# yandooo/cilium

Measured on AMD Instinct MI355X. Metric: L7 verdicts/sec + scanned GB/s (HBM roofline frac), 1/2/4/8 MI355X, higher is better.
Workload: dtype u8

## Files before the change

cilium_amd/_lib.py:

```python
import ctypes as C
import os

HERE = os.path.dirname(os.path.abspath(__file__))
LIB_PATH = os.environ.get("L7G_LIB") or os.path.join(HERE, "libl7gpu.so")

DENY, ALLOW, PARSE_ERROR, INCOMPLETE, UNSUPPORTED = 0, 1, 2, 3, 4
PROTO_HTTP, PROTO_KAFKA, PROTO_MEMCACHE, PROTO_R2D2, PROTO_CASSANDRA = 1, 2, 3, 4, 5
VERDICT_NAMES = {DENY: "DENY", ALLOW: "ALLOW", PARSE_ERROR: "PARSE_ERROR",
                 INCOMPLETE: "INCOMPLETE", UNSUPPORTED: "UNSUPPORTED"}


class Conn(C.Structure):
    _fields_ = [("policy", C.c_int32), ("port", C.c_uint32), ("ingress", C.c_uint8),
                ("proto", C.c_uint8), ("flags", C.c_uint16), ("src_id", C.c_uint32),
                ("dst_id", C.c_uint32)]


class Stats(C.Structure):
    _fields_ = [(n, C.c_uint32) for n in (
        "policies", "rules", "http_rulesets", "http_chunks", "http_dfas", "http_dfa_states",
        "kafka_rulesets", "kafka_rules", "kafka_topics")] + [
        ("table_bytes", C.c_uint64), ("http_image_bytes", C.c_uint64), ("hot_ruleset", C.c_int32),
        ("hot_image_bytes", C.c_uint32)] + [
        (n, C.c_uint32) for n in ("mc_rulesets", "mc_rules", "mc_dfas", "mc_dfa_states", "http_nfas", "mc_nfas")] + [
        ("nfa_pool_bytes", C.c_uint64), ("r2d2_rulesets", C.c_uint32), ("r2d2_rules", C.c_uint32)]


EXPORTS = (
    "l7g_engine_create", "l7g_engine_destroy", "l7g_policy_update", "l7g_policy_index",
    "l7g_policy_nrules", "l7g_conns_set", "l7g_conn_update", "l7g_classify", "l7g_classify_host", "l7g_stats",
    "l7g_debug_regex", "l7g_debug_phase_times", "l7g_profile_enable", "l7g_profile_last",
    "l7g_debug_kafka_phase_times", "l7g_debug_frame_phase_times", "l7g_kafka_deny_response", "l7g_debug_regex_nfa", "l7g_policy_update_proto", "l7g_kafka_corr_create", "l7g_kafka_corr_destroy",
    "l7g_kafka_corr_requests", "l7g_kafka_corr_responses", "l7g_kafka_corr_gc", "l7g_kafka_corr_size",
    "l7g_flow_stats_enable", "l7g_flow_stats",
    "l7g_tables_export", "l7g_tables_import", "l7g_tables_compiled", "l7g_tables_digest",
    "l7g_frame_streams", "l7g_classify_streams", "l7g_service_enable", "l7g_service_stats",
    "l7g_cass_sessions_enable", "l7g_cass_replies", "l7g_cass_replies_host", "l7g_cass_session_reset",
    "l7g_cass_session_stats",
    "l7g_classify_logged", "l7g_classify_logged_host", "l7g_kafka_api_key_name",
    "l7g_deny_replies", "l7g_deny_replies_host", "l7g_deny_reply_template",
)


class FlowStat(C.Structure):
    _fields_ = [("policy", C.c_int32), ("proto", C.c_uint8), ("ingress", C.c_uint8), ("port", C.c_uint16),
                ("received", C.c_uint64), ("forwarded", C.c_uint64), ("denied", C.c_uint64), ("error", C.c_uint64)]


class Span(C.Structure):
    _fields_ = [("off", C.c_uint32), ("len", C.c_uint32)]


class _LogHttp(C.Structure):
    _fields_ = [(n, C.c_uint32) for n in ("method_len", "path_len", "host_off", "host_len", "head_len", "nheaders")]


class _LogKafka(C.Structure):
    _fields_ = [("api_version", C.c_int16), ("pad", C.c_int16), ("correlation_id", C.c_int32),
                ("ntopics", C.c_uint32)]


class _LogUnion(C.Union):
    _fields_ = [("http", _LogHttp), ("kafka", _LogKafka)]


class LogRec(C.Structure):
    _fields_ = [("kind", C.c_uint8), ("flags", C.c_uint8), ("api_key", C.c_int16), ("u", _LogUnion),
                ("reserved", C.c_uint32)]


class LogOut(C.Structure):
    _fields_ = [("rec", C.c_void_p), ("topics", C.c_void_p), ("topic_stride", C.c_uint32)]

# ... 53 lines not shown
    lib.l7g_service_stats.argtypes = [vp, C.POINTER(C.c_uint64)]
    lib.l7g_service_stats.restype = None
    lib.l7g_stats.argtypes = [vp, C.POINTER(Stats)]
    lib.l7g_debug_regex.argtypes = [cp, sz, C.c_int, cp, sz, cp, sz]
    lib.l7g_debug_regex_nfa.argtypes = [cp, sz, C.c_int, cp, sz, cp, sz]
    lib.l7g_debug_phase_times.argtypes = [vp, vp, C.c_int]
    lib.l7g_debug_kafka_phase_times.argtypes = [vp, vp, C.c_int]
    lib.l7g_debug_frame_phase_times.argtypes = [vp, vp, C.c_int]
    lib.l7g_kafka_corr_create.restype = vp
    lib.l7g_kafka_corr_destroy.argtypes = [vp]
    lib.l7g_kafka_corr_requests.argtypes = [vp, vp, vp, vp, C.c_uint32, vp]
    lib.l7g_kafka_corr_responses.argtypes = [vp, vp, vp, vp, C.c_uint32, vp]
    lib.l7g_kafka_corr_gc.restype = C.c_uint64
    lib.l7g_kafka_corr_gc.argtypes = [vp, C.c_uint64]
    lib.l7g_kafka_corr_size.restype = C.c_uint64
    lib.l7g_kafka_corr_size.argtypes = [vp]
    lib.l7g_kafka_deny_response.argtypes = [cp, sz, vp, sz, C.POINTER(C.c_size_t)]
    lib.l7g_profile_enable.argtypes = [vp, C.c_int]
    lib.l7g_flow_stats_enable.argtypes = [vp, C.c_int]
    lib.l7g_flow_stats.argtypes = [vp, vp, C.c_uint32, C.POINTER(C.c_uint32), C.c_int]
    lib.l7g_profile_last.argtypes = [vp, vp]
    if hasattr(lib, "l7g_classify_logged"):
        lib.l7g_classify_logged.argtypes = [vp, vp, C.c_uint64, vp, vp, vp, C.c_uint32, vp, vp, vp, vp,
                                            C.POINTER(LogOut), vp]
        lib.l7g_classify_logged_host.argtypes = [vp, vp, C.c_uint64, vp, vp, vp, C.c_uint32, vp, vp, vp,
                                                 C.POINTER(LogOut)]
        lib.l7g_kafka_api_key_name.restype = cp
        lib.l7g_kafka_api_key_name.argtypes = [C.c_int16]
    if hasattr(lib, "l7g_deny_replies"):
        lib.l7g_deny_replies.argtypes = [vp, vp, C.c_uint64, vp, vp, vp, C.c_uint32, vp, C.POINTER(ReplyOut), vp]
        lib.l7g_deny_replies_host.argtypes = [vp, vp, C.c_uint64, vp, vp, vp, C.c_uint32, vp, C.POINTER(ReplyOut)]
        lib.l7g_deny_reply_template.restype = vp
        lib.l7g_deny_reply_template.argtypes = [C.c_int, C.POINTER(C.c_size_t)]
    _libs[path] = lib
    return lib


def debug_regex(pattern, data, anchored=True, nfa=False):
    lib = load()
    p = pattern.encode() if isinstance(pattern, str) else pattern
    d = data.encode() if isinstance(data, str) else data
    err = C.create_string_buffer(512)
    fn = lib.l7g_debug_regex_nfa if nfa else lib.l7g_debug_regex
    r = fn(p, len(p), 1 if anchored else 0, d, len(d), err, 512)
    if r < 0:
        raise ValueError(err.value.decode(errors="replace"))
    return bool(r)


def kafka_api_key_name(key):
    r = load().l7g_kafka_api_key_name(int(key))
    return r.decode() if r is not None else None


def deny_reply_template(proto):
    n = C.c_size_t(0)
    p = load().l7g_deny_reply_template(int(proto), C.byref(n))
    return C.string_at(p, n.value) if p else b""


def kafka_deny_response(req):
    lib = load()
    cap = 4 * len(req) + 256
    out = C.create_string_buffer(cap)
    n = C.c_size_t(0)
    rc = lib.l7g_kafka_deny_response(req, len(req), out, cap, C.byref(n))
    if rc == -1:
        return None
# ... 40 lines not shown
```

cilium_amd/csrc/capi.cc:

```cpp
#include <algorithm>
#include <cstring>

#include "engine/nfa_pool.h"
#include "engine_state.h"
#include "policy/npds_proto.h"
#include "regex/nfa_walk.h"
#include "regex/re_dfa.h"

namespace {

void set_err(char *err, size_t errlen, const std::string &m) {
    if (!err || errlen == 0) return;
    size_t n = std::min(errlen - 1, m.size());
    memcpy(err, m.data(), n);
    err[n] = 0;
}

template <class T>
size_t Put(std::vector<uint8_t> &blob, const std::vector<T> &v) {
    size_t off = (blob.size() + 255) & ~(size_t)255;
    blob.resize(off + v.size() * sizeof(T) + 16);
    if (!v.empty()) memcpy(blob.data() + off, v.data(), v.size() * sizeof(T));
    return off;
}
// ... 132 lines not shown
        std::vector<uint8_t> blob;
        const BlobLayout L = AssembleBlob(e, blob);
        const HttpImage &H = e->hc->image();
        const KafkaImage &K = e->kc->image();
        const McImage &M = e->mc->image();
        const R2Image &R = e->r2->image();
        const CassImage &CI = e->cs->image();
        uint8_t *d = nullptr;
        if ((rc = hipMalloc(&d, blob.size())) != hipSuccess) return rc;
        if ((rc = hipMemcpy(d, blob.data(), blob.size(), hipMemcpyHostToDevice)) != hipSuccess) { hipFree(d); return rc; }
        if (e->d_blob) { WaitLastClassify(e); hipFree(e->d_blob); }
        e->d_blob = d;
        e->blob_bytes = blob.size();
        HttpTables &T = e->ht;
        T.rulesets = (const DevRuleset *)(d + L.o_rs);
        T.images = d + L.o_img;
        T.nrulesets = (uint32_t)H.rulesets.size();
        T.hot_ruleset = e->hot_ruleset;
        T.nfa_pool = H.nfa_pool.empty() ? nullptr : d + L.o_nfa;
        T.nfa_bits = nullptr;
        auto lane_words = [](uint32_t w) { return w > (uint32_t)kNfaMaxWords ? 2 * w : 0u; };
        T.nfa_scratch = nullptr;
        T.nfa_lane_words = lane_words(e->hc->nfa_max_words());
        KafkaTables &KT = e->kt;
        KT.rulesets = (const DevKafkaRuleset *)(d + L.k_rs);
        KT.rules = (const DevKafkaRule *)(d + L.k_r);
        KT.index = (const uint32_t *)(d + L.k_idx);
        KT.topic_hash = (const DevStrSlot *)(d + L.k_th);
        KT.client_hash = (const DevStrSlot *)(d + L.k_ch);
        KT.strings = (const uint8_t *)(d + L.k_s);
        KT.nrulesets = (uint32_t)K.rulesets.size();
        KT.topic_mask = K.topic_mask;
        KT.client_mask = K.client_mask;
        McTables &MT = e->mt;
        MT.rulesets = (const DevRuleset *)(d + L.m_rs);
        MT.images = d + L.m_img;
        MT.nrulesets = (uint32_t)M.rulesets.size();
        MT.images_len = (uint32_t)M.images.size();
        MT.nfa_pool = M.nfa_pool.empty() ? nullptr : d + L.m_nfa;
        MT.max_chunks = (uint32_t)M.max_chunks;
        MT.nfa_scratch = nullptr;
        MT.nfa_lane_words = lane_words(e->mc->nfa_max_words());
        R2Tables &RT = e->rt;
        RT.rulesets = (const DevRuleset *)(d + L.r_rs);
        RT.images = d + L.r_img;
        RT.nrulesets = (uint32_t)R.rulesets.size();
        RT.nfa_pool = R.nfa_pool.empty() ? nullptr : d + L.r_nfa;
        RT.nfa_scratch = nullptr;
        RT.nfa_lane_words = lane_words(e->r2->nfa_max_words());
        CassTables &CT = e->ct;
        CT.rulesets = (const DevRuleset *)(d + L.c_rs);
        CT.images = d + L.c_img;
        CT.nrulesets = (uint32_t)CI.rulesets.size();
        CT.nfa_pool = CI.nfa_pool.empty() ? nullptr : d + L.c_nfa;
        CT.lower = (const uint32_t *)(d + L.c_low);
        CT.nlower = (uint32_t)(CI.lower.size() / 2);
        CT.nfa_scratch = nullptr;
        CT.nfa_lane_words = lane_words(e->cs->nfa_max_words());
        e->tables_dirty = false;
    }
    if (e->conns_dirty) {
        if ((rc = WaitLastClassify(e)) != hipSuccess) return rc;
        size_t need = std::max<size_t>(e->conns.size(), 1);
        if (need > e->conns_cap) {
            if (e->d_conns) { hipFree(e->d_conns); e->d_conns = nullptr; }
            if ((rc = hipMalloc(&e->d_conns, need * sizeof(DevConn))) != hipSuccess) return rc;
// ... 408 lines not shown
    return (int)rc;
}

int l7g_profile_last(l7g_engine *e, float out_ms[4]) {
    std::lock_guard<std::mutex> g(e->mu);
    for (int k = 0; k < 4; k++) out_ms[k] = 0.f;
    bool any = false;
    for (auto &kv : e->scr) any = any || kv.second->launched;
    if (!e->profile || !any) return (int)hipErrorNotReady;
    hipError_t rc = hipEventSynchronize(e->prof_ev[4]);
    for (int k = 0; k < 4 && rc == hipSuccess; k++)
        if (e->prof_ran[k]) rc = hipEventElapsedTime(&out_ms[k], e->prof_ev[k], e->prof_ev[k + 1]);
    return (int)rc;
}

int l7g_debug_phase_times(l7g_engine *e, uint64_t *out16, int reset) {
    if (!e || e->device < 0) return (int)hipErrorNoDevice;
    hipSetDevice(e->device);
    return (int)HttpPhaseTimes(out16, reset != 0);
}

int l7g_debug_frame_phase_times(l7g_engine *e, uint64_t *out8, int reset) {
    if (!e || e->device < 0) return (int)hipErrorNoDevice;
    hipSetDevice(e->device);
    return (int)FramePhaseTimes(out8, reset != 0);
}

int l7g_debug_kafka_phase_times(l7g_engine *e, uint64_t *out8, int reset) {
    if (!e || e->device < 0) return (int)hipErrorNoDevice;
    hipSetDevice(e->device);
    return (int)KafkaPhaseTimes(out8, reset != 0);
}

int l7g_debug_regex(const char *pat, size_t patlen, int anchored, const uint8_t *s, size_t slen, char *err,
                    size_t errlen) {
    std::string m;
    auto ast = re::Parse(std::string(pat, patlen), &m);
    if (!ast) { set_err(err, errlen, m); return -1; }
    re::DFA d;
    std::vector<re::Pattern> ps{{ast.get(), anchored != 0}};
    if (!re::BuildDFA(ps, 1 << 16, &d, &m)) { set_err(err, errlen, m); return -1; }
    auto acc = re::RunDFA(d, s, slen);
    return (int)(acc[0] & 1);
}

int l7g_debug_regex_nfa(const char *pat, size_t patlen, int anchored, const uint8_t *s, size_t slen, char *err,
                        size_t errlen) {
    std::string m;
    auto ast = re::Parse(std::string(pat, patlen), &m);
    if (!ast) { set_err(err, errlen, m); return -1; }
    re::BitNfa n;
    if (!re::BuildBitNfa({ast.get(), anchored != 0}, kNfaMaxPositions, &n, &m, kNfaMaxWords)) {
        set_err(err, errlen, m);
        return -1;
    }
    std::vector<uint8_t> pool;
    const uint64_t off = AppendDevNfa(n, &pool, &m);
    if (off == ~0ull) { set_err(err, errlen, m); return -1; }
    std::vector<uint64_t> scratch(2 * (size_t)n.W);
    return nfa_run(pool.data(), off, s, (uint32_t)slen, scratch.data()) ? 1 : 0;
}

}
```

cilium_amd/csrc/device_tables.h:

```cpp
#pragma once
#include <stddef.h>
#include <stdint.h>

#if defined(__HIPCC__)
#define L7_HD __host__ __device__
#else
#define L7_HD
#endif

namespace l7 {

enum : uint8_t {
    V_DENY = 0, V_ALLOW = 1, V_PARSE_ERROR = 2, V_INCOMPLETE = 3, V_UNSUPPORTED = 4,
};
enum : uint8_t { PROTO_NONE = 0, PROTO_HTTP = 1, PROTO_KAFKA = 2, PROTO_MEMCACHE = 3, PROTO_R2D2 = 4, PROTO_CASSANDRA = 5 };
#define L7_PROTO_OWNED(p) ((p) >= PROTO_HTTP && (p) <= PROTO_CASSANDRA)

#ifndef L7_KAFKA_CLASSES
#define L7_KAFKA_CLASSES 8
#endif

constexpr int kCntWords = 32;
constexpr int kCntMc = L7_KAFKA_CLASSES;
constexpr int kCntHttp = L7_KAFKA_CLASSES + 2;
// ... 133 lines not shown
    uint64_t nfa;
    uint32_t mask_off;
    uint8_t slot;
    uint8_t pad[3];
};

struct DevRuleset {
    uint32_t image_off;
    uint32_t image_len;
};

struct HttpTables {
    const DevRuleset *rulesets;
    const uint8_t *images;
    uint32_t nrulesets;
    int32_t hot_ruleset;
    const uint8_t *nfa_pool;
    uint64_t *nfa_bits;
    uint64_t *nfa_scratch;
    uint32_t nfa_lane_words;
};

struct DevKafkaRule {
    uint64_t keymask;
    int32_t client;
    int32_t gid;
    int16_t version;
    uint8_t any_key;
    uint8_t has_version;
    uint8_t has_topic;
    uint8_t pad[3];
};
static_assert(sizeof(DevKafkaRule) == 24, "DevKafkaRule layout");
struct DevKafkaTopicEnt {
    uint32_t p0;
    uint32_t off, cnt;
    uint32_t pad;
    DevKafkaRule r0;
    uint32_t pad2[2];
};
static_assert(sizeof(DevKafkaTopicEnt) == 48, "DevKafkaTopicEnt layout");
struct DevKafkaRuleset {
    uint32_t rule_first, nrules;
    uint32_t topicless_off, ntopicless;
    uint32_t topics_off, ntopics;
    uint32_t bykey_off;
    uint32_t tdense_off;
    uint8_t any;
    uint8_t pad[3];
};
struct DevStrSlot {
    uint32_t hash;
    uint32_t str_off;
    uint16_t len;
    uint16_t used;
    int32_t id;
    uint32_t pre[4];
};
static_assert(sizeof(DevStrSlot) == 32, "DevStrSlot layout");
constexpr uint32_t kWHashSeed = 0x811C9DC5u;
L7_HD inline uint32_t l7_whash_step(uint32_t h, uint32_t w) {
    h = (h ^ w) * 0x9E3779B1u;
    return h ^ (h >> 15);
}
L7_HD inline uint32_t l7_whash_final(uint32_t h, uint32_t n) {
    h = (h ^ n) * 0x85EBCA6Bu;
    return h ^ (h >> 13);
}

struct KafkaTables {
    const DevKafkaRuleset *rulesets;
    const DevKafkaRule *rules;
    const uint32_t *index;
    const DevStrSlot *topic_hash;
    const DevStrSlot *client_hash;
    const uint8_t *strings;
    uint32_t nrulesets;
    uint32_t topic_mask, client_mask;
    uint32_t pad;
};

constexpr int kMcTextRows = 32;
constexpr int kMcMaxChunks = 4;
constexpr int kMcMaxDfas = 4;
struct McImgHeader {
    uint8_t nchunks;
    uint8_t terminal;
    uint8_t ndfa;
    uint8_t pad0;
    uint32_t text_off;
    uint32_t op_off;
    uint32_t empty_off;
    uint32_t nopred_off;
    uint32_t rule_off;
    uint32_t dfa_off;
    uint32_t owned_off;
    uint32_t nfa_off;
    uint32_t nnfa;
    uint32_t pad1[6];
};
static_assert(sizeof(McImgHeader) == 64, "McImgHeader layout");
constexpr uint32_t kMcDfaOff = sizeof(McImgHeader);

struct McTables {
    const DevRuleset *rulesets;
    const uint8_t *images;
    uint32_t nrulesets;
    uint32_t images_len;
    const uint8_t *nfa_pool;
    uint32_t max_chunks;
    uint32_t nfa_lane_words;
    uint64_t *nfa_scratch;
// ... 97 lines not shown
```

cilium_amd/csrc/engine/kafka_compile.cc:

```cpp
#include "kafka_compile.h"

#include <algorithm>
#include <cstring>

namespace l7 {

uint32_t KafkaStrHash(const uint8_t *s, size_t n) {
    uint32_t h = kWHashSeed;
    for (size_t i = 0; i < n; i += 4) {
        uint32_t w = 0;
        for (size_t k = 0; k < 4 && i + k < n; k++) w |= (uint32_t)s[i + k] << (8 * k);
        h = l7_whash_step(h, w);
    }
    return l7_whash_final(h, (uint32_t)n);
}

namespace {
void BuildHash(const std::unordered_map<std::string, int> &ids, std::vector<uint8_t> &strings,
               std::vector<DevStrSlot> &table, uint32_t &mask) {
    size_t cap = 16;
    while (cap < ids.size() * 2 + 2) cap <<= 1;
    table.assign(cap, DevStrSlot{});
    mask = (uint32_t)(cap - 1);
    std::vector<const std::string *> byid(ids.size());
    for (auto &kv : ids) byid[kv.second] = &kv.first;
    for (size_t id = 0; id < byid.size(); id++) {
        const std::string &s = *byid[id];
        uint32_t h = KafkaStrHash((const uint8_t *)s.data(), s.size());
        uint32_t slot = h & mask;
        while (table[slot].used) slot = (slot + 1) & mask;
        DevStrSlot &d = table[slot];
        d.hash = h;
        d.len = (uint16_t)s.size();
        d.used = 1;
        d.id = (int32_t)id;
// ... 29 lines not shown
    if (policy >= 0 && policy < (int)ps_->policies.size()) {
        const PortPolicy *ex, *wc;
        ps_->policies[policy].Lookup(ingress, port, &ex, &wc);
        for (const PortPolicy *pp : {ex, wc}) {
            if (!pp) continue;
            if (proxylib) {
                if (!pp->px_installed) continue;
                if (!pp->px_have_l7 || pp->rules.empty()) { rules.push_back(&kWildcard); any = true; continue; }
                for (auto &r : pp->rules) {
                    if (!r.RemoteOk(src_id)) continue;
                    if (r.NumL7() == 0) { rules.push_back(&kWildcard); any = true; }
                    else if (r.type == PortRule::Kafka) { for (auto &k : r.kafka) rules.push_back(&k); any = true; }
                }
                continue;
            }
            for (auto &r : pp->rules) {
                if (!r.RemoteOk(src_id)) continue;
                if (r.type == PortRule::Kafka) { for (auto &k : r.kafka) rules.push_back(&k); any = true; }
                else if (r.type == PortRule::None) { rules.push_back(&kWildcard); any = true; }
            }
        }
    }
    std::vector<int> key;
    for (auto *r : rules) key.push_back(r == &kWildcard ? -1 : r->id);
    auto ck = std::make_pair(key, (int)any);
    auto it = cache_.find(ck);
    if (it != cache_.end()) return it->second;
    int id = Compile(rules, any);
    cache_.emplace(ck, id);
    return id;
}

static constexpr size_t kDenseTopicBudget = size_t(64) << 20;

int KafkaCompiler::Compile(const std::vector<const KafkaRule *> &rules, bool any) {
    compiled++;
    KafkaImage &I = img_;
    DevKafkaRuleset rs{};
    rs.any = any ? 1 : 0;
    rs.rule_first = (uint32_t)I.rules.size();
    rs.nrules = (uint32_t)rules.size();
    std::map<int, std::vector<uint32_t>> by_topic;
    std::vector<uint32_t> topicless;
    std::vector<std::vector<uint32_t>> bykey(65);
    for (uint32_t pos = 0; pos < rules.size(); pos++) {
        const KafkaRule &k = *rules[pos];
        DevKafkaRule d{};
        d.keymask = k.keymask;
        d.any_key = k.any_key ? 1 : 0;
        d.has_version = k.has_version ? 1 : 0;
        d.version = k.version;
        d.has_topic = k.topic.empty() ? 0 : 1;
        d.client = k.client.empty() ? -1 : client_id_.at(k.client);
        d.gid = k.id;
        I.rules.push_back(d);
        if (k.topic.empty()) topicless.push_back(pos);
        else by_topic[topic_id_.at(k.topic)].push_back(pos);
        for (int key = 0; key < 64; key++)
            if (k.any_key || ((k.keymask >> key) & 1)) bykey[key].push_back(pos);
        if (k.any_key) bykey[64].push_back(pos);
    }
    rs.topicless_off = (uint32_t)I.index.size();
    rs.ntopicless = (uint32_t)topicless.size();
    I.index.insert(I.index.end(), topicless.begin(), topicless.end());
    std::vector<uint32_t> dir;
    for (auto &kv : by_topic) {
        dir.push_back((uint32_t)kv.first);
        dir.push_back((uint32_t)I.index.size());
        dir.push_back((uint32_t)kv.second.size());
        I.index.insert(I.index.end(), kv.second.begin(), kv.second.end());
    }
    rs.topics_off = (uint32_t)I.index.size();
    rs.ntopics = (uint32_t)by_topic.size();
    I.index.insert(I.index.end(), dir.begin(), dir.end());
    rs.tdense_off = ~0u;
    constexpr size_t kEntU32 = sizeof(DevKafkaTopicEnt) / 4;
    if (!by_topic.empty() && I.index.size() + 3 + kEntU32 * I.ntopics <= kDenseTopicBudget) {
        I.index.resize((I.index.size() + 3) & ~(size_t)3, 0);
        rs.tdense_off = (uint32_t)I.index.size();
        I.index.resize(I.index.size() + kEntU32 * I.ntopics, 0);
        for (size_t t = 0; t < dir.size(); t += 3) {
            DevKafkaTopicEnt e{};
            e.off = dir[t + 1];
            e.cnt = dir[t + 2];
            e.p0 = I.index[e.off];
            e.r0 = I.rules[rs.rule_first + e.p0];
            memcpy(&I.index[rs.tdense_off + kEntU32 * dir[t]], &e, sizeof e);
        }
    }
    std::vector<uint32_t> keydir;
    for (auto &l : bykey) {
        keydir.push_back((uint32_t)I.index.size() + 0);
        keydir.push_back((uint32_t)l.size());
    }
    for (size_t k = 0; k < bykey.size(); k++) {
        keydir[2 * k] = (uint32_t)I.index.size();
        I.index.insert(I.index.end(), bykey[k].begin(), bykey[k].end());
    }
    rs.bykey_off = (uint32_t)I.index.size();
    I.index.insert(I.index.end(), keydir.begin(), keydir.end());
    I.rulesets.push_back(rs);
    return (int)I.rulesets.size() - 1;
}

}
```

cilium_amd/csrc/engine/kafka_compile.h:

```cpp
#pragma once
#include <cstdint>
#include <map>
#include <string>
#include <unordered_map>
#include <vector>

#include "../device_tables.h"
#include "../policy/policy.h"
#include "serial.h"

namespace l7 {

struct KafkaImage {
    std::vector<DevKafkaRuleset> rulesets;
    std::vector<DevKafkaRule> rules;
    std::vector<uint32_t> index;
    std::vector<DevStrSlot> topic_hash, client_hash;
    std::vector<uint8_t> strings;
    uint32_t topic_mask = 0, client_mask = 0;
    size_t ntopics = 0;
};

class KafkaCompiler {
public:
    explicit KafkaCompiler(const PolicySet *ps);
    int RulesetFor(int policy, bool ingress, uint32_t port, uint64_t src_id, bool proxylib, std::string *err);
    const KafkaImage &image() const { return img_; }

    void Save(Ser &s) const {
        s.vec(img_.rulesets); s.vec(img_.rules); s.vec(img_.index); s.vec(img_.topic_hash); s.vec(img_.client_hash);
        s.vec(img_.strings); s.u64(img_.topic_mask); s.u64(img_.client_mask); s.u64(img_.ntopics);
        s.umap(topic_id_); s.umap(client_id_); s.cache(cache_);
    }
    bool Load(Des &d) {
        d.vec(img_.rulesets); d.vec(img_.rules); d.vec(img_.index); d.vec(img_.topic_hash); d.vec(img_.client_hash);
        d.vec(img_.strings); img_.topic_mask = (uint32_t)d.u64(); img_.client_mask = (uint32_t)d.u64();
        img_.ntopics = d.u64();
        d.umap(topic_id_); d.umap(client_id_); d.cache(cache_);
        auto table_ok = [](const std::vector<DevStrSlot> &t, uint32_t mask) {
            return !t.empty() && (uint64_t)mask + 1 == t.size() && (t.size() & (t.size() - 1)) == 0;
        };
        if (!d.ok || !table_ok(img_.topic_hash, img_.topic_mask) || !table_ok(img_.client_hash, img_.client_mask))
            return false;
        for (const auto &r : img_.rulesets)
            if ((uint64_t)r.rule_first + r.nrules > img_.rules.size()) return false;
        return true;
    }
    size_t compiled = 0;

private:
    const PolicySet *ps_;
    KafkaImage img_;
    std::unordered_map<std::string, int> topic_id_, client_id_;
    std::map<std::pair<std::vector<int>, int>, int> cache_;
    int Compile(const std::vector<const KafkaRule *> &rules, bool any);
};

uint32_t KafkaStrHash(const uint8_t *s, size_t n);

}
```

cilium_amd/csrc/kernels/kafka_classify.hip:

```cpp
#include <hip/hip_runtime.h>

#include "../device_tables.h"
#include "kafka_dec.h"
#include "launch.h"

namespace l7 {

namespace {

constexpr int kBlock = 256;


__device__ __forceinline__ uint32_t le_load4(Cur &c, const uint8_t *p) {
    const uintptr_t a = (uintptr_t)p;
    const uint32_t k = (uint32_t)(a & 15);
    if (k <= 12) {
        cur_fill(c, a);
        const uint32_t w0 = c.w0, w1 = c.w1, w2 = c.w2, w3 = c.w3;
        const uint32_t i = k >> 2;
        const uint32_t lo = i == 0 ? w0 : i == 1 ? w1 : i == 2 ? w2 : w3;
        const uint32_t hi = i == 0 ? w1 : i == 1 ? w2 : i == 2 ? w3 : 0u;
        return __builtin_amdgcn_alignbyte(hi, lo, k & 3);
    }
    uint32_t v = 0;
// ... 317 lines not shown
            np = kd_arraylen(d, false, bad);
            if (bad) { rc = -1; break; }
            for (int32_t p = 0; p < np && !d.err; p++) {
                kd_skip(d, 4); kd_skip(d, 8);
                if (ver == 1) kd_skip(d, 8);
                uint32_t o2, l2;
                kd_string(d, o2, l2);
            }
        }
        break;
    case 9:
        kd_string(d, o, l);
        nt = kd_arraylen(d, true, bad);
        if (bad) { rc = -1; break; }
        for (int32_t t = 0; t < nt && !d.err; t++) {
            kd_string(d, o, l);
            h.topic(o, l);
            np = kd_arraylen(d, false, bad);
            if (bad) { rc = -1; break; }
            if (kd_bulk(d, np, 4u)) continue;
            for (int32_t p = 0; p < np && !d.err; p++) kd_skip(d, 4);
        }
        break;
    case 10:
        kd_string(d, o, l);
        if (ver >= 1) kd_skip(d, 1);
        break;
    }
    if (rc == 0 && d.err) rc = -1;
    return rc;
}

template <class R>
__device__ __forceinline__ int32_t str_lookup(const DevStrSlot *tab, uint32_t mask, const uint8_t *strings, R &r,
                                              uint32_t pos, uint32_t n) {
    uint32_t h = kWHashSeed;
    uint32_t p0 = 0, p1 = 0, p2 = 0, p3 = 0;
    for (uint32_t i = 0; i < n; i += 4) {
        const uint32_t rem = n - i;
        const uint32_t keep = rem >= 4 ? 0xFFFFFFFFu : (1u << (8 * rem)) - 1u;
        const uint32_t w = r.le4(pos + i) & keep;
        h = l7_whash_step(h, w);
        p0 = i == 0 ? w : p0;
        p1 = i == 4 ? w : p1;
        p2 = i == 8 ? w : p2;
        p3 = i == 12 ? w : p3;
    }
    h = l7_whash_final(h, n);
    for (uint32_t slot = h & mask;; slot = (slot + 1) & mask) {
        const DevStrSlot e = tab[slot];
        if (!e.used) return -1;
        if (e.hash == h && e.len == n) {
            bool eq = e.pre[0] == p0 && e.pre[1] == p1 && e.pre[2] == p2 && e.pre[3] == p3;
            const uint32_t *t = reinterpret_cast<const uint32_t *>(strings + e.str_off);
            for (uint32_t i = 16; i < n && eq; i += 4) {
                const uint32_t rem = n - i;
                const uint32_t keep = rem >= 4 ? 0xFFFFFFFFu : (1u << (8 * rem)) - 1u;
                eq = t[i >> 2] == (r.le4(pos + i) & keep);
            }
            if (eq) return e.id;
        }
    }
}

struct ReqInfo {
    int kind;
    int version;
    int typed;
    int32_t client;
};

__device__ __forceinline__ bool rule_matches(const DevKafkaRule &r, const ReqInfo &q) {
    if (!r.any_key && (q.kind < 0 || q.kind > 63 || !((r.keymask >> q.kind) & 1))) return false;
    if (r.has_version && r.version != q.version) return false;
    if (!r.has_topic && r.client < 0) return true;
    if (q.typed == 1) return r.client < 0 || r.client == q.client;
    if (q.typed == 2) return true;
    return !(r.has_topic && is_topic_api_key(q.kind));
}

__device__ __forceinline__ uint32_t topic_first(const KafkaTables &T, const DevKafkaRuleset &rs, const ReqInfo &q,
                                                int32_t tid) {
    if (tid < 0 || rs.ntopics == 0) return kInf;
    uint32_t off, cnt;
    if (rs.tdense_off != ~0u) {
        const uint4 *ep = reinterpret_cast<const uint4 *>(T.index + rs.tdense_off +
                                                          (uint32_t)(sizeof(DevKafkaTopicEnt) / 4) * (uint32_t)tid);
        const uint4 e0 = ep[0], e1 = ep[1], e2 = ep[2];
        off = e0.y;
        cnt = e0.z;
        if (cnt == 0) return kInf;
        DevKafkaRule r0;
        const uint32_t w[6] = {e1.x, e1.y, e1.z, e1.w, e2.x, e2.y};
        __builtin_memcpy(&r0, w, sizeof r0);
        if (rule_matches(r0, q)) return e0.x;
        for (uint32_t i = 1; i < cnt; i++) {
            const uint32_t p = T.index[off + i];
            if (rule_matches(T.rules[rs.rule_first + p], q)) return p;
        }
        return kInf;
    } else {
        const uint32_t *dir = T.index + rs.topics_off;
        uint32_t lo = 0, hi = rs.ntopics;
        while (lo < hi) {
            const uint32_t m = (lo + hi) >> 1;
            if (dir[3 * m] < (uint32_t)tid) lo = m + 1; else hi = m;
        }
        if (lo >= rs.ntopics || dir[3 * lo] != (uint32_t)tid) return kInf;
        off = dir[3 * lo + 1];
        cnt = dir[3 * lo + 2];
    }
    for (uint32_t i = 0; i < cnt; i++) {
        const uint32_t p = T.index[off + i];
        if (rule_matches(T.rules[rs.rule_first + p], q)) return p;
    }
    return kInf;
}

__device__ __forceinline__ uint32_t matches_rule(const KafkaTables &T, const DevKafkaRuleset &rs, const ReqInfo &q,
                                                 uint32_t ntopics, uint32_t cmax) {
    uint32_t best = kInf;
    if (ntopics == 0) {
        const int key = (q.kind >= 0 && q.kind < 64) ? q.kind : 64;
        const uint32_t off = T.index[rs.bykey_off + 2 * key], cnt = T.index[rs.bykey_off + 2 * key + 1];
        for (uint32_t i = 0; i < cnt; i++) {
            const uint32_t p = T.index[off + i];
            if (rule_matches(T.rules[rs.rule_first + p], q)) { best = p; break; }
        }
    } else {
        for (uint32_t i = 0; i < rs.ntopicless; i++) {
            const uint32_t p = T.index[rs.topicless_off + i];
            if (p >= cmax) break;
            if (rule_matches(T.rules[rs.rule_first + p], q)) { best = p; break; }
        }
        if (best == kInf) best = cmax;
    }
    return best;
}

struct NoTopicLog {};
struct TopicLog {
    LogSpan *row;
    uint32_t stride;
};
template <class L>
struct ExactHooks {
    const KafkaTables &T;
    const DevKafkaRuleset &rs;
    ReqInfo &q;
    GRd &r;
    const uint32_t *crctab;
    uint8_t *stage;
    uint32_t ntopics, cmax;
    L log;
    __device__ __forceinline__ void client(uint32_t o, uint32_t l) {
        q.client = str_lookup(T.client_hash, T.client_mask, T.strings, r, o, l);
        if (q.client < 0) q.client = -2;
    }
    __device__ __forceinline__ void topic(uint32_t o, uint32_t l) {
        if (q.typed != 1) return;
        if constexpr (!std::is_same<L, NoTopicLog>::value) {
            if (ntopics < log.stride) log.row[ntopics] = LogSpan{o, l};
        }
        ntopics++;
        const int32_t tid = l > 0 ? str_lookup(T.topic_hash, T.topic_mask, T.strings, r, o, l) : -1;
        const uint32_t e = topic_first(T, rs, q, tid);
        cmax = cmax > e ? cmax : e;
    }
    __device__ __forceinline__ bool msg(uint32_t pos, uint32_t n, uint32_t stored) {
        r.hlim = 0;
        return crc32_ieee_staged(crctab, r.cur, r.b + pos, n, stage, r.lastc) == stored;
    }
    __device__ __forceinline__ bool msg_win(uint32_t pos, uint32_t n, uint32_t stored) {
        return crc32_ieee_window(crctab, r.cur, r.b + pos, n, stage, r.lastc) == stored;
    }
};

}

template <int kWaves, bool kLog>
__global__ __launch_bounds__(kBlock) __attribute__((amdgpu_waves_per_eu(kWaves, 8))) void kafka_classify_kernel(
    Batch B, KafkaTables T, const uint32_t *__restrict__ sel, const uint32_t *__restrict__ sel_count,
    uint32_t answer_other, uint32_t *__restrict__ zlist, uint32_t *__restrict__ zcount, uint32_t *__restrict__ work,
    uint32_t main_sweep, LogRec *__restrict__ lrec, LogSpan *__restrict__ ltopics, uint32_t lstride) {
    const uint32_t n = B.n, nconns = B.nconns;
    static_assert(kBlock >= 256, "one CRC table entry per thread");
    __shared__ uint32_t crctab[kCrcTables * 256];
    __shared__ __attribute__((aligned(16))) uint8_t crcstage[kBlock / 64][4096];
    uint8_t *stage = crcstage[threadIdx.x >> 6];
    crc_tables_init(crctab, threadIdx.x);
    constexpr int kCls = L7_KAFKA_CLASSES;
    uint32_t kc[kCls] = {n};
    uint32_t m = n;
    if (sel) {
        m = 0;
        for (int c = 0; c < kCls; c++) { kc[c] = sel_count[c]; m += kc[c]; }
    }
    const uint32_t stride = main_sweep ? main_sweep : gridDim.x * kBlock;
    auto next_entry = [&](uint32_t i) -> uint32_t {
        if (!work) return i + stride;
        const uint32_t lane = threadIdx.x & 63;
        uint32_t t = 0;
        if (lane == (uint32_t)__builtin_amdgcn_readfirstlane(lane)) t = atomicAdd(work, 64u);
        return stride + __builtin_amdgcn_readfirstlane(t) + lane;
    };
    for (uint32_t i = main_sweep ? next_entry(0) : blockIdx.x * kBlock + threadIdx.x; i < m; i = next_entry(i)) {
        uint32_t idx = i;
        if (sel) {
            uint32_t c = 0, j = i;
            bool hit = false;
#pragma unroll
            for (int k = kCls - 1; k > 0; k--) {
                if (!hit) {
// ... 8 lines not shown
        const uint64_t off = B.offs[idx];
        const uint32_t len = B.lens[idx];
        uint8_t verdict = V_PARSE_ERROR;
        int32_t rule = -1;
        uint32_t consumed = 0;
        bool zflag = false;
        if (conn.proto != PROTO_KAFKA || conn.ruleset < 0 || (uint32_t)conn.ruleset >= T.nrulesets) {
            if (!answer_other || (L7_PROTO_OWNED(conn.proto) && conn.proto != PROTO_KAFKA)) continue;
            verdict = V_UNSUPPORTED;
        }
        do {
            if (verdict == V_UNSUPPORTED) break;
            if (!l7_in_arena(off, len, B.arena_len)) { verdict = V_UNSUPPORTED; break; }
            if (len < 4) { verdict = V_INCOMPLETE; break; }
            GRd r{B.arena + off, ((uintptr_t)(B.arena + off) + len - 1) & ~(uintptr_t)15, {}, stage, 0};
            r.stage_head();
            r.cur.line = ~(uintptr_t)0;
            const int32_t size = (int32_t)r.be(0, 4);
            if (size <= 0) break;
            if (len < 6) { verdict = V_INCOMPLETE; break; }
            if ((uint64_t)(uint32_t)size + 4 > kMaxParseBuf) break;
            const uint32_t rawlen = (uint32_t)size + 4;
            if (rawlen > len) { verdict = V_INCOMPLETE; break; }
            if (rawlen < 12) break;
            ReqInfo q;
            q.kind = (int16_t)r.be(4, 2);
            q.version = (int16_t)r.be(6, 2);
            q.typed = kind_typed(q.kind);
            q.client = -2;
            const DevKafkaRuleset &rs = T.rulesets[conn.ruleset];
            using Log = typename std::conditional<kLog, TopicLog, NoTopicLog>::type;
            Log lg{};
            if constexpr (kLog) lg = TopicLog{ltopics + (size_t)idx * lstride, lstride};
            ExactHooks<Log> h{T, rs, q, r, crctab, stage, 0, 0, lg};
            if (q.typed && kafka_walk(r, rawlen, q.kind, zflag, h) == -1) break;
            consumed = rawlen;
            verdict = V_DENY;
            if constexpr (kLog) {
                const uint32_t corr = (uint32_t)r.be(8, 4);
                uint4 *o = reinterpret_cast<uint4 *>(lrec + idx);
                o[0] = make_uint4(LOG_KAFKA | (h.ntopics > lstride ? 0x100u : 0u) | ((uint32_t)(uint16_t)q.kind << 16),
                                  (uint32_t)(uint16_t)q.version, corr, h.ntopics);
                o[1] = make_uint4(0, 0, 0, 0);
            }
            if (!rs.any) break;
            const uint32_t best = matches_rule(T, rs, q, h.ntopics, h.cmax);
            if (best != kInf) { verdict = V_ALLOW; rule = T.rules[rs.rule_first + best].gid; }
        } while (false);
        B.verdict[idx] = verdict;
        B.rule[idx] = rule;
        B.consumed[idx] = consumed;
        if (zflag && zlist && (verdict == V_ALLOW || verdict == V_DENY)) zlist[atomicAdd(zcount, 1u)] = idx;
    }
}

hipError_t KafkaPhaseTimes(uint64_t *, bool) { return hipErrorNotSupported; }

hipError_t LaunchKafkaClassify(const Batch &B, const KafkaTables &T, const uint32_t *sel, const uint32_t *sel_count,
                               bool answer_other, uint32_t *zlist, uint32_t *zcount, uint32_t *work,
                               hipStream_t stream, int leave_per_cu, bool helper, const LogOut *log) {
    if (B.n == 0) return hipSuccess;
    uint32_t blocks = (B.n + kBlock - 1) / kBlock;
    const bool beside = leave_per_cu > 0;
    if (helper && (!beside || !work)) return hipErrorInvalidValue;
    const bool lg = log != nullptr;
    const auto kernel = lg ? kafka_classify_kernel<4, true>
                           : (beside ? kafka_classify_kernel<6, false> : kafka_classify_kernel<5, false>);
    static int cus[2][2] = {}, per_cu[2][2] = {};
    if (cus[lg][beside] == 0) {
        int dev = 0, c = 0, p = 0;
        if (hipGetDevice(&dev) == hipSuccess &&
            hipDeviceGetAttribute(&c, hipDeviceAttributeMultiprocessorCount, dev) == hipSuccess &&
            hipOccupancyMaxActiveBlocksPerMultiprocessor(&p, kernel, kBlock, 0) == hipSuccess && c > 0 && p > 0) {
            per_cu[lg][beside] = p;
            cus[lg][beside] = c;
        } else {
            per_cu[lg][beside] = 32;
            cus[lg][beside] = 256;
        }
    }
    const int pc = per_cu[lg][beside], ncu = cus[lg][beside];
    const int slots = beside && pc > leave_per_cu ? pc - leave_per_cu : pc;
    if (!work) blocks = blocks > 8192 ? 8192 : blocks;
    else if (blocks > (uint32_t)(ncu * slots)) blocks = (uint32_t)(ncu * slots);
    const uint32_t grid = helper ? min(blocks, (uint32_t)(ncu * min(leave_per_cu, pc))) : blocks;
    const uint32_t main_sweep = helper ? blocks * (uint32_t)kBlock : 0u;
    LogRec *lrec = lg ? log->rec : nullptr;
    LogSpan *ltopics = lg ? log->topics : nullptr;
    hipLaunchKernelGGL(kernel, dim3(grid), dim3(kBlock), 0, stream, B, T, sel, sel_count, answer_other ? 1u : 0u, zlist,
                       zcount, work, main_sweep, lrec, ltopics, lg ? log->stride : 0u);
    return hipGetLastError();
}

}
```

include/l7gpu.h:

```cpp
#ifndef L7GPU_H
#define L7GPU_H
#include <stddef.h>
#include <stdint.h>

#ifdef __cplusplus
extern "C" {
#endif

typedef struct l7g_engine l7g_engine;

enum { L7G_PROTO_HTTP = 1, L7G_PROTO_KAFKA = 2, L7G_PROTO_MEMCACHE = 3, L7G_PROTO_R2D2 = 4, L7G_PROTO_CASSANDRA = 5 };
enum {
    L7G_DENY = 0,
    L7G_ALLOW = 1,
    L7G_PARSE_ERROR = 2,
    L7G_INCOMPLETE = 3,
    L7G_UNSUPPORTED = 4,
};

enum { L7G_CONN_MC_TEXT = 1, L7G_CONN_MC_BINARY = 2, L7G_CONN_PROXYLIB = 4 };

typedef struct {
    int32_t policy;
    uint32_t port;
// ... 106 lines not shown
int l7g_batcher_submit(l7g_batcher *b, const uint8_t *req, uint32_t len, uint32_t conn, l7g_done_fn done, void *ctx);
int l7g_batcher_flush(l7g_batcher *b);
void l7g_batcher_destroy(l7g_batcher *b);
void l7g_batcher_stats(l7g_batcher *b, uint64_t *requests, uint64_t *launches);
void l7g_batcher_timing(l7g_batcher *b, uint64_t out[5]);

int l7g_profile_enable(l7g_engine *e, int on);

typedef struct {
    int32_t policy;
    uint8_t proto;
    uint8_t ingress;
    uint16_t port;
    uint64_t received, forwarded, denied, error;
} l7g_flow_stat_t;
int l7g_flow_stats_enable(l7g_engine *e, int on);
int l7g_flow_stats(l7g_engine *e, l7g_flow_stat_t *out, uint32_t cap, uint32_t *n, int reset);
int l7g_profile_last(l7g_engine *e, float out_ms[4]);

int l7g_debug_phase_times(l7g_engine *e, uint64_t *out16, int reset);
int l7g_debug_kafka_phase_times(l7g_engine *e, uint64_t *out8, int reset);
int l7g_debug_frame_phase_times(l7g_engine *e, uint64_t *out8, int reset);

typedef struct l7g_kafka_corr l7g_kafka_corr;
l7g_kafka_corr *l7g_kafka_corr_create(void);
void l7g_kafka_corr_destroy(l7g_kafka_corr *c);
int l7g_kafka_corr_requests(l7g_kafka_corr *c, uint8_t *arena, const uint64_t *off, const uint32_t *len, uint32_t n,
                            uint32_t *new_ids);
int l7g_kafka_corr_responses(l7g_kafka_corr *c, uint8_t *arena, const uint64_t *off, const uint32_t *len, uint32_t n,
                             uint8_t *found);
uint64_t l7g_kafka_corr_gc(l7g_kafka_corr *c, uint64_t lifetime_ms);
uint64_t l7g_kafka_corr_size(l7g_kafka_corr *c);

int l7g_debug_regex(const char *pat, size_t patlen, int anchored, const uint8_t *s, size_t slen, char *err,
                    size_t errlen);
int l7g_debug_regex_nfa(const char *pat, size_t patlen, int anchored, const uint8_t *s, size_t slen, char *err,
                        size_t errlen);

#ifdef __cplusplus
}
#endif
#endif
```

Before: 2.994 billion.

## Replace global topic lookup plus dense per-ruleset table with fused per-ruleset topic hash

Kafka topic matching used to hash the topic name into a global topic-id table and then index a dense per-ruleset entry array sized by the total topic count. Each ruleset now gets its own open-addressed 64-byte-slot hash table that holds the hash, length, string prefix and the first rule, so one probe both identifies the topic and yields its rule. The aim is fewer dependent global-memory loads per topic and less table memory. The binary-search directory path is kept only through a template flag when some ruleset has no table, and a debug budget knob plus validation of the table on import are added.

Measured after the change: 3.005 billion (median of 6 runs). No clear change (+0.4%).

```diff
diff --git a/cilium_amd/_lib.py b/cilium_amd/_lib.py
--- a/cilium_amd/_lib.py
+++ b/cilium_amd/_lib.py
@@ -39,6 +39,7 @@
     "l7g_cass_session_stats",
     "l7g_classify_logged", "l7g_classify_logged_host", "l7g_kafka_api_key_name",
     "l7g_deny_replies", "l7g_deny_replies_host", "l7g_deny_reply_template",
+    "l7g_debug_kafka_topic_budget",
 )
 
 
@@ -158,8 +159,15 @@
         lib.l7g_deny_replies_host.argtypes = [vp, vp, C.c_uint64, vp, vp, vp, C.c_uint32, vp, C.POINTER(ReplyOut)]
         lib.l7g_deny_reply_template.restype = vp
         lib.l7g_deny_reply_template.argtypes = [C.c_int, C.POINTER(C.c_size_t)]
+    if hasattr(lib, "l7g_debug_kafka_topic_budget"):
+        lib.l7g_debug_kafka_topic_budget.restype = None
+        lib.l7g_debug_kafka_topic_budget.argtypes = [C.c_uint64]
     _libs[path] = lib
     return lib
+
+
+def debug_kafka_topic_budget(words):
+    load().l7g_debug_kafka_topic_budget(int(words))
 
 
 def debug_regex(pattern, data, anchored=True, nfa=False):
diff --git a/cilium_amd/csrc/capi.cc b/cilium_amd/csrc/capi.cc
--- a/cilium_amd/csrc/capi.cc
+++ b/cilium_amd/csrc/capi.cc
@@ -188,6 +188,9 @@
         KT.nrulesets = (uint32_t)K.rulesets.size();
         KT.topic_mask = K.topic_mask;
         KT.client_mask = K.client_mask;
+        KT.has_dir = 0;
+        for (const DevKafkaRuleset &r : K.rulesets)
+            if (r.ntopics != 0 && r.ttab_off == ~0u) KT.has_dir = 1;
         McTables &MT = e->mt;
         MT.rulesets = (const DevRuleset *)(d + L.m_rs);
         MT.images = d + L.m_img;
@@ -662,6 +665,8 @@
     return (int)KafkaPhaseTimes(out8, reset != 0);
 }
 
+void l7g_debug_kafka_topic_budget(uint64_t words) { SetTopicTableBudget((size_t)words); }
+
 int l7g_debug_regex(const char *pat, size_t patlen, int anchored, const uint8_t *s, size_t slen, char *err,
                     size_t errlen) {
     std::string m;
diff --git a/cilium_amd/csrc/device_tables.h b/cilium_amd/csrc/device_tables.h
--- a/cilium_amd/csrc/device_tables.h
+++ b/cilium_amd/csrc/device_tables.h
@@ -189,23 +189,28 @@
     uint8_t pad[3];
 };
 static_assert(sizeof(DevKafkaRule) == 24, "DevKafkaRule layout");
-struct DevKafkaTopicEnt {
+struct DevKafkaTopicSlot {
+    uint32_t hash;
+    uint16_t len;
+    uint16_t used;
+    uint32_t str_off;
     uint32_t p0;
+    uint32_t pre[4];
     uint32_t off, cnt;
-    uint32_t pad;
     DevKafkaRule r0;
-    uint32_t pad2[2];
-};
-static_assert(sizeof(DevKafkaTopicEnt) == 48, "DevKafkaTopicEnt layout");
+};
+static_assert(sizeof(DevKafkaTopicSlot) == 64, "DevKafkaTopicSlot layout");
+constexpr uint32_t kTopicSlotU32 = sizeof(DevKafkaTopicSlot) / 4;
 struct DevKafkaRuleset {
     uint32_t rule_first, nrules;
     uint32_t topicless_off, ntopicless;
     uint32_t topics_off, ntopics;
     uint32_t bykey_off;
-    uint32_t tdense_off;
+    uint32_t ttab_off, ttab_mask;
     uint8_t any;
     uint8_t pad[3];
 };
+static_assert(sizeof(DevKafkaRuleset) == 40, "DevKafkaRuleset layout");
 struct DevStrSlot {
     uint32_t hash;
     uint32_t str_off;
@@ -234,7 +239,7 @@
     const uint8_t *strings;
     uint32_t nrulesets;
     uint32_t topic_mask, client_mask;
-    uint32_t pad;
+    uint32_t has_dir;
 };
 
 constexpr int kMcTextRows = 32;
diff --git a/cilium_amd/csrc/engine/kafka_compile.cc b/cilium_amd/csrc/engine/kafka_compile.cc
--- a/cilium_amd/csrc/engine/kafka_compile.cc
+++ b/cilium_amd/csrc/engine/kafka_compile.cc
@@ -1,6 +1,7 @@
 #include "kafka_compile.h"
 
 #include <algorithm>
+#include <atomic>
 #include <cstring>
 
 namespace l7 {
@@ -96,6 +97,33 @@
 }
 
 static constexpr size_t kDenseTopicBudget = size_t(64) << 20;
+static std::atomic<size_t> g_topic_budget{kDenseTopicBudget};
+size_t TopicTableBudget() { return g_topic_budget.load(std::memory_order_relaxed); }
+void SetTopicTableBudget(size_t words) {
+    g_topic_budget.store(words == 0 || words > kDenseTopicBudget ? kDenseTopicBudget : words, std::memory_order_relaxed);
+}
+
+bool KafkaCompiler::TopicTableOk(const DevKafkaRuleset &r) const {
+    const KafkaImage &I = img_;
+    if (r.ttab_off == ~0u) return r.ttab_mask == ~0u;
+    const uint64_t cap = (uint64_t)r.ttab_mask + 1;
+    if (r.ttab_mask == ~0u || (cap & (cap - 1)) != 0 || r.ttab_off % 16 != 0 ||
+        (uint64_t)r.ttab_off + kTopicSlotU32 * cap > I.index.size())
+        return false;
+    uint64_t used = 0;
+    for (uint64_t s = 0; s < cap; s++) {
+        DevKafkaTopicSlot e;
+        memcpy(&e, &I.index[r.ttab_off + kTopicSlotU32 * s], sizeof e);
+        if (!e.used) continue;
+        used++;
+        if (e.str_off % 4 != 0 || (uint64_t)e.str_off + ((e.len + 3u) & ~3u) > I.strings.size()) return false;
+        if (e.cnt == 0 || (uint64_t)e.off + e.cnt > I.index.size()) return false;
+        for (uint32_t i = 0; i < e.cnt; i++)
+            if (I.index[e.off + i] >= r.nrules) return false;
+        if (e.p0 != I.index[e.off]) return false;
+    }
+    return 2 * used <= cap;
+}
 
 int KafkaCompiler::Compile(const std::vector<const KafkaRule *> &rules, bool any) {
     compiled++;
@@ -137,19 +165,36 @@
     rs.topics_off = (uint32_t)I.index.size();
     rs.ntopics = (uint32_t)by_topic.size();
     I.index.insert(I.index.end(), dir.begin(), dir.end());
-    rs.tdense_off = ~0u;
-    constexpr size_t kEntU32 = sizeof(DevKafkaTopicEnt) / 4;
-    if (!by_topic.empty() && I.index.size() + 3 + kEntU32 * I.ntopics <= kDenseTopicBudget) {
-        I.index.resize((I.index.size() + 3) & ~(size_t)3, 0);
-        rs.tdense_off = (uint32_t)I.index.size();
-        I.index.resize(I.index.size() + kEntU32 * I.ntopics, 0);
+    rs.ttab_off = rs.ttab_mask = ~0u;
+    size_t cap = 2;
+    while (cap < 2 * by_topic.size()) cap <<= 1;
+    if (!by_topic.empty() && I.index.size() + 15 + kTopicSlotU32 * cap <= TopicTableBudget()) {
+        I.index.resize((I.index.size() + 15) & ~(size_t)15, 0);
+        rs.ttab_off = (uint32_t)I.index.size();
+        rs.ttab_mask = (uint32_t)(cap - 1);
+        I.index.resize(I.index.size() + kTopicSlotU32 * cap, 0);
+        auto slot_at = [&](uint32_t s) { return &I.index[rs.ttab_off + kTopicSlotU32 * (size_t)s]; };
         for (size_t t = 0; t < dir.size(); t += 3) {
-            DevKafkaTopicEnt e{};
+            const std::string &name = rules[I.index[dir[t + 1]]]->topic;
+            const uint32_t h = KafkaStrHash((const uint8_t *)name.data(), name.size());
+            uint32_t g = h & I.topic_mask;
+            while (I.topic_hash[g].used && I.topic_hash[g].id != (int32_t)dir[t]) g = (g + 1) & I.topic_mask;
+            const DevStrSlot &src = I.topic_hash[g];
+            if (!src.used) continue;
+            DevKafkaTopicSlot e{};
+            e.hash = src.hash;
+            e.len = src.len;
+            e.used = 1;
+            e.str_off = src.str_off;
+            memcpy(e.pre, src.pre, sizeof e.pre);
             e.off = dir[t + 1];
             e.cnt = dir[t + 2];
             e.p0 = I.index[e.off];
             e.r0 = I.rules[rs.rule_first + e.p0];
-            memcpy(&I.index[rs.tdense_off + kEntU32 * dir[t]], &e, sizeof e);
+            uint32_t s = h & rs.ttab_mask;
+            DevKafkaTopicSlot cur;
+            while (memcpy(&cur, slot_at(s), sizeof cur), cur.used) s = (s + 1) & rs.ttab_mask;
+            memcpy(slot_at(s), &e, sizeof e);
         }
     }
     std::vector<uint32_t> keydir;
diff --git a/cilium_amd/csrc/engine/kafka_compile.h b/cilium_amd/csrc/engine/kafka_compile.h
--- a/cilium_amd/csrc/engine/kafka_compile.h
+++ b/cilium_amd/csrc/engine/kafka_compile.h
@@ -43,7 +43,7 @@
         if (!d.ok || !table_ok(img_.topic_hash, img_.topic_mask) || !table_ok(img_.client_hash, img_.client_mask))
             return false;
         for (const auto &r : img_.rulesets)
-            if ((uint64_t)r.rule_first + r.nrules > img_.rules.size()) return false;
+            if ((uint64_t)r.rule_first + r.nrules > img_.rules.size() || !TopicTableOk(r)) return false;
         return true;
     }
     size_t compiled = 0;
@@ -54,8 +54,11 @@
     std::unordered_map<std::string, int> topic_id_, client_id_;
     std::map<std::pair<std::vector<int>, int>, int> cache_;
     int Compile(const std::vector<const KafkaRule *> &rules, bool any);
+    bool TopicTableOk(const DevKafkaRuleset &r) const;
 };
 
 uint32_t KafkaStrHash(const uint8_t *s, size_t n);
+size_t TopicTableBudget();
+void SetTopicTableBudget(size_t words);
 
 }
diff --git a/cilium_amd/csrc/kernels/kafka_classify.hip b/cilium_amd/csrc/kernels/kafka_classify.hip
--- a/cilium_amd/csrc/kernels/kafka_classify.hip
+++ b/cilium_amd/csrc/kernels/kafka_classify.hip
@@ -373,10 +373,10 @@
 }
 
 template <class R>
-__device__ __forceinline__ int32_t str_lookup(const DevStrSlot *tab, uint32_t mask, const uint8_t *strings, R &r,
-                                              uint32_t pos, uint32_t n) {
+__device__ __forceinline__ uint32_t str_hash(R &r, uint32_t pos, uint32_t n, uint32_t &p0, uint32_t &p1, uint32_t &p2,
+                                             uint32_t &p3) {
     uint32_t h = kWHashSeed;
-    uint32_t p0 = 0, p1 = 0, p2 = 0, p3 = 0;
+    p0 = p1 = p2 = p3 = 0;
     for (uint32_t i = 0; i < n; i += 4) {
         const uint32_t rem = n - i;
         const uint32_t keep = rem >= 4 ? 0xFFFFFFFFu : (1u << (8 * rem)) - 1u;
@@ -387,19 +387,30 @@
         p2 = i == 8 ? w : p2;
         p3 = i == 12 ? w : p3;
     }
-    h = l7_whash_final(h, n);
+    return l7_whash_final(h, n);
+}
+template <class R>
+__device__ __forceinline__ bool str_tail_eq(const uint32_t *t, R &r, uint32_t pos, uint32_t n) {
+    bool eq = true;
+    for (uint32_t i = 16; i < n && eq; i += 4) {
+        const uint32_t rem = n - i;
+        const uint32_t keep = rem >= 4 ? 0xFFFFFFFFu : (1u << (8 * rem)) - 1u;
+        eq = t[i >> 2] == (r.le4(pos + i) & keep);
+    }
+    return eq;
+}
+
+template <class R>
+__device__ __forceinline__ int32_t str_lookup(const DevStrSlot *tab, uint32_t mask, const uint8_t *strings, R &r,
+                                              uint32_t pos, uint32_t n) {
+    uint32_t p0, p1, p2, p3;
+    const uint32_t h = str_hash(r, pos, n, p0, p1, p2, p3);
     for (uint32_t slot = h & mask;; slot = (slot + 1) & mask) {
         const DevStrSlot e = tab[slot];
         if (!e.used) return -1;
         if (e.hash == h && e.len == n) {
-            bool eq = e.pre[0] == p0 && e.pre[1] == p1 && e.pre[2] == p2 && e.pre[3] == p3;
-            const uint32_t *t = reinterpret_cast<const uint32_t *>(strings + e.str_off);
-            for (uint32_t i = 16; i < n && eq; i += 4) {
-                const uint32_t rem = n - i;
-                const uint32_t keep = rem >= 4 ? 0xFFFFFFFFu : (1u << (8 * rem)) - 1u;
-                eq = t[i >> 2] == (r.le4(pos + i) & keep);
-            }
-            if (eq) return e.id;
+            const bool eq = e.pre[0] == p0 && e.pre[1] == p1 && e.pre[2] == p2 && e.pre[3] == p3;
+            if (eq && str_tail_eq(reinterpret_cast<const uint32_t *>(strings + e.str_off), r, pos, n)) return e.id;
         }
     }
 }
@@ -423,39 +434,46 @@
 __device__ __forceinline__ uint32_t topic_first(const KafkaTables &T, const DevKafkaRuleset &rs, const ReqInfo &q,
                                                 int32_t tid) {
     if (tid < 0 || rs.ntopics == 0) return kInf;
-    uint32_t off, cnt;
-    if (rs.tdense_off != ~0u) {
-        const uint4 *ep = reinterpret_cast<const uint4 *>(T.index + rs.tdense_off +
-                                                          (uint32_t)(sizeof(DevKafkaTopicEnt) / 4) * (uint32_t)tid);
-        const uint4 e0 = ep[0], e1 = ep[1], e2 = ep[2];
-        off = e0.y;
-        cnt = e0.z;
-        if (cnt == 0) return kInf;
+    const uint32_t *dir = T.index + rs.topics_off;
+    uint32_t lo = 0, hi = rs.ntopics;
+    while (lo < hi) {
+        const uint32_t m = (lo + hi) >> 1;
+        if (dir[3 * m] < (uint32_t)tid) lo = m + 1; else hi = m;
+    }
+    if (lo >= rs.ntopics || dir[3 * lo] != (uint32_t)tid) return kInf;
+    const uint32_t off = dir[3 * lo + 1], cnt = dir[3 * lo + 2];
+    for (uint32_t i = 0; i < cnt; i++) {
+        const uint32_t p = T.index[off + i];
+        if (rule_matches(T.rules[rs.rule_first + p], q)) return p;
+    }
+    return kInf;
+}
+
+template <class R>
+__device__ __forceinline__ uint32_t topic_fused(const KafkaTables &T, const DevKafkaRuleset &rs, const ReqInfo &q,
+                                                R &r, uint32_t pos, uint32_t n) {
+    uint32_t p0, p1, p2, p3;
+    const uint32_t h = str_hash(r, pos, n, p0, p1, p2, p3);
+    const uint32_t mask = rs.ttab_mask;
+    const uint4 *tab = reinterpret_cast<const uint4 *>(T.index + rs.ttab_off);
+    for (uint32_t slot = h & mask;; slot = (slot + 1) & mask) {
+        const uint4 *ep = tab + (size_t)slot * (sizeof(DevKafkaTopicSlot) / 16);
+        const uint4 e0 = ep[0], e1 = ep[1], e2 = ep[2], e3 = ep[3];
+        if ((e0.y >> 16) == 0) return kInf;
+        if (e0.x != h || (e0.y & 0xFFFFu) != n) continue;
+        const bool eq = e1.x == p0 && e1.y == p1 && e1.z == p2 && e1.w == p3;
+        if (!eq || !str_tail_eq(reinterpret_cast<const uint32_t *>(T.strings + e0.z), r, pos, n)) continue;
         DevKafkaRule r0;
-        const uint32_t w[6] = {e1.x, e1.y, e1.z, e1.w, e2.x, e2.y};
+        const uint32_t w[6] = {e2.z, e2.w, e3.x, e3.y, e3.z, e3.w};
         __builtin_memcpy(&r0, w, sizeof r0);
-        if (rule_matches(r0, q)) return e0.x;
+        if (rule_matches(r0, q)) return e0.w;
+        const uint32_t off = e2.x, cnt = e2.y;
         for (uint32_t i = 1; i < cnt; i++) {
             const uint32_t p = T.index[off + i];
             if (rule_matches(T.rules[rs.rule_first + p], q)) return p;
         }
         return kInf;
-    } else {
-        const uint32_t *dir = T.index + rs.topics_off;
-        uint32_t lo = 0, hi = rs.ntopics;
-        while (lo < hi) {
-            const uint32_t m = (lo + hi) >> 1;
-            if (dir[3 * m] < (uint32_t)tid) lo = m + 1; else hi = m;
-        }
-        if (lo >= rs.ntopics || dir[3 * lo] != (uint32_t)tid) return kInf;
-        off = dir[3 * lo + 1];
-        cnt = dir[3 * lo + 2];
-    }
-    for (uint32_t i = 0; i < cnt; i++) {
-        const uint32_t p = T.index[off + i];
-        if (rule_matches(T.rules[rs.rule_first + p], q)) return p;
-    }
-    return kInf;
+    }
 }
 
 __device__ __forceinline__ uint32_t matches_rule(const KafkaTables &T, const DevKafkaRuleset &rs, const ReqInfo &q,
@@ -484,7 +502,7 @@
     LogSpan *row;
     uint32_t stride;
 };
-template <class L>
+template <class L, bool kDir>
 struct ExactHooks {
     const KafkaTables &T;
     const DevKafkaRuleset &rs;
@@ -504,8 +522,13 @@
             if (ntopics < log.stride) log.row[ntopics] = LogSpan{o, l};
         }
         ntopics++;
-        const int32_t tid = l > 0 ? str_lookup(T.topic_hash, T.topic_mask, T.strings, r, o, l) : -1;
-        const uint32_t e = topic_first(T, rs, q, tid);
+        uint32_t e = kInf;
+        if (rs.ttab_off != ~0u) {
+            if (l > 0) e = topic_fused(T, rs, q, r, o, l);
+        } else if constexpr (kDir) {
+            const int32_t tid = l > 0 ? str_lookup(T.topic_hash, T.topic_mask, T.strings, r, o, l) : -1;
+            e = topic_first(T, rs, q, tid);
+        }
         cmax = cmax > e ? cmax : e;
     }
     __device__ __forceinline__ bool msg(uint32_t pos, uint32_t n, uint32_t stored) {
@@ -519,7 +542,7 @@
 
 }
 
-template <int kWaves, bool kLog>
+template <int kWaves, bool kLog, bool kDir>
 __global__ __launch_bounds__(kBlock) __attribute__((amdgpu_waves_per_eu(kWaves, 8))) void kafka_classify_kernel(
     Batch B, KafkaTables T, const uint32_t *__restrict__ sel, const uint32_t *__restrict__ sel_count,
     uint32_t answer_other, uint32_t *__restrict__ zlist, uint32_t *__restrict__ zcount, uint32_t *__restrict__ work,
@@ -594,7 +617,7 @@
             using Log = typename std::conditional<kLog, TopicLog, NoTopicLog>::type;
             Log lg{};
             if constexpr (kLog) lg = TopicLog{ltopics + (size_t)idx * lstride, lstride};
-            ExactHooks<Log> h{T, rs, q, r, crctab, stage, 0, 0, lg};
+            ExactHooks<Log, kDir> h{T, rs, q, r, crctab, stage, 0, 0, lg};
             if (q.typed && kafka_walk(r, rawlen, q.kind, zflag, h) == -1) break;
             consumed = rawlen;
             verdict = V_DENY;
@@ -626,9 +649,15 @@
     const bool beside = leave_per_cu > 0;
     if (helper && (!beside || !work)) return hipErrorInvalidValue;
     const bool lg = log != nullptr;
-    const auto kernel = lg ? kafka_classify_kernel<4, true>
-                           : (beside ? kafka_classify_kernel<6, false> : kafka_classify_kernel<5, false>);
-    static int cus[2][2] = {}, per_cu[2][2] = {};
+    const bool dir = T.has_dir != 0;
+    const auto kernel =
+        dir ? (lg ? kafka_classify_kernel<4, true, true>
+                  : (beside ? kafka_classify_kernel<6, false, true> : kafka_classify_kernel<5, false, true>))
+            : (lg ? kafka_classify_kernel<4, true, false>
+                  : (beside ? kafka_classify_kernel<6, false, false> : kafka_classify_kernel<5, false, false>));
+    static int cus_[2][2][2] = {}, per_cu_[2][2][2] = {};
+    auto &cus = cus_[dir];
+    auto &per_cu = per_cu_[dir];
     if (cus[lg][beside] == 0) {
         int dev = 0, c = 0, p = 0;
         if (hipGetDevice(&dev) == hipSuccess &&
diff --git a/include/l7gpu.h b/include/l7gpu.h
--- a/include/l7gpu.h
+++ b/include/l7gpu.h
@@ -162,6 +162,8 @@
 uint64_t l7g_kafka_corr_gc(l7g_kafka_corr *c, uint64_t lifetime_ms);
 uint64_t l7g_kafka_corr_size(l7g_kafka_corr *c);
 
+void l7g_debug_kafka_topic_budget(uint64_t words);
+
 int l7g_debug_regex(const char *pat, size_t patlen, int anchored, const uint8_t *s, size_t slen, char *err,
                     size_t errlen);
 int l7g_debug_regex_nfa(const char *pat, size_t patlen, int anchored, const uint8_t *s, size_t slen, char *err,
```
